# RyanXLi/OneshotDet

Measured on AMD Instinct MI355X. Metric: images/sec/GPU fwd+bwd, 800x1024 target + 127x127 query, bs=8; 1->8 GPU scaling, higher is better.
Workload: dtype bf16; 1 GPU; BASELINE.json configs[2]: bs=8/GPU, 800x1024 target + 127x127 query, bf16 MFMA convs, forward (two R-50-FPN backbones, query pooling, correlation, FCOS head, training proposals) + FCOS loss + backward (stem/layer1 frozen) + gradient all-reduce + SGD(momentum) + weight repack; global_batch=8, parallelism=dp1: one rank, no collective anywhere in the step, world_size=1

## Files before the change

include/oneshotdet_hip.h:

```cpp
#ifndef ONESHOTDET_HIP_H
#define ONESHOTDET_HIP_H

#include <stdint.h>

#ifdef __cplusplus
extern "C" {
#endif

#define OSD_F32 0
#define OSD_BF16 1

#define OSD_OK 0
#define OSD_ERR_INVALID_ARG (-1)
#define OSD_ERR_UNSUPPORTED (-2)
#define OSD_ERR_LAUNCH (-3)
#define OSD_ERR_WORKSPACE (-4)

#define OSD_ACT_NONE 0
#define OSD_ACT_RELU 1
#define OSD_ACT_EXP_SCALE 2

#define OSD_RES_NONE 0
#define OSD_RES_SAME 1
#define OSD_RES_UP2X 2
// ... 118 lines not shown
int osd_sigmoid_focal_bwd(const float* logits, const int32_t* targets, const float* d_losses, float* d_logits, int m,
                          int classes, float gamma, float alpha, void* stream);

int osd_pack_conv_weight_dgrad(const float* w, const float* scale, void* dst, int cout, int cin, int r, int s, int rows,
                               int cout_pad, int src_orsi, int dtype, void* stream);
int osd_conv2d_wgrad(const osd_conv_desc* d, const void* x, const void* dy, const float* scale, float* dw, float* db,
                     void* stream);
int osd_conv2d_wgrad_grouped(const osd_conv_desc* d, int n_seg, const void* const* xs, const void* const* dys,
                             const int32_t* ns, const int32_t* hs, const int32_t* ws, const float* scale, float* dw,
                             float* db, void* stream);
int osd_conv2d_wgrad_pred(const osd_conv_desc* d, int n_seg, const void* const* xs, const void* const* dys, const int32_t* ns,
                          const int32_t* hs, const int32_t* ws, float* dw, float* db, void* workspace, void* stream);
int64_t osd_conv2d_wgrad_pred_workspace_bytes(int n_seg, const int32_t* ns, const int32_t* hs, const int32_t* ws, int cin);
int osd_pred_dy_gather(const osd_conv_desc* d, int n_seg, const void* const* dys, const int32_t* ns, const int32_t* hs,
                       const int32_t* ws, void* g, void* stream);
int osd_pred_dgrad_pack(int dtype, const float* w, int cout, int cin, void* wd, void* stream);
int osd_conv2d_wgrad_pred_gathered(const osd_conv_desc* d, int n_seg, const void* const* xs, const void* g, const int32_t* ns,
                                   const int32_t* hs, const int32_t* ws, float* dw, float* db, void* workspace, void* stream);
int osd_conv2d_wgrad_batched(const osd_conv_desc* d, int n_seg, const void* const* xs, const void* const* dys,
                             const float* const* scales, float* const* dws, float* const* dbs, void* stream);
int osd_conv2d_wgrad_multi(const osd_conv_desc* d, int n_seg, const void* const* xs, const void* const* dys,
                           const int32_t* ns, const int32_t* hs, const int32_t* ws, const float* const* scales,
                           float* const* dws, float* const* dbs, void* stream);
int osd_conv2d_wgrad_mixed(int n_seg, const osd_conv_desc* descs, const void* const* xs, const void* const* dys,
                           const float* const* scales, float* const* dws, float* const* dbs, void* stream);
int osd_unpack_wgrad(const float* dw_packed, const float* scale, float* grad_oihw, int cout, int cin, int r, int s,
                     int accumulate, void* stream);
int osd_bias_grad(const void* dy, float* db, int m, int c, int stride, int dtype, void* stream);
int osd_conv2d_dgrad_naive(const osd_conv_desc* d, const void* dy, const void* w_fwd_packed, const void* mask,
                           const void* addend, void* dx, void* stream);
int osd_scatter2x(const void* src, const void* mask, const void* addend, void* dst, int n, int h, int w, int ho, int wo,
                  int c, int dtype, void* stream);
int osd_add_mask(const void* a, const void* b, const void* mask, void* out, int64_t numel, int dtype, void* stream);
int osd_upsample2x_bwd(const void* inner, const void* prev, void* top, int n, int h, int w, int c, int dtype, void* stream);
int osd_correlate_bwd_query(const void* g, const void* feat, float* dq, int n, int hw, int c, int dtype, void* stream);
int osd_correlate_bwd_query_levels(int n_levels, const void* const* gs, const void* const* feats, float* const* dqs,
                                   const int32_t* hws, int n, int c, int dtype, void* stream);
int osd_roialign_bwd(const float* gy, const float* rois, float* gx, int b, int h, int w, int c, int num_rois,
                     float spatial_scale, int ph, int pw, int sampling_ratio, void* stream);
int osd_shot_mean_bwd(const float* gy, float* gx, int b, int shots, int c, void* stream);
int osd_query_pool_levels_bwd(int n_levels, const float* const* dqs, const int32_t* hs, const int32_t* ws, const float* scales,
                              const float* rois, int batch, int shots, int c, int sampling_ratio, float* gx32, void* const* outs,
                              int dtype, void* stream);
int osd_query_avgpool_levels_bwd(int n_levels, const float* const* dqs, const int32_t* hs, const int32_t* ws, int batch,
                                 int shots, int c, void* const* outs, int dtype, void* stream);
int osd_cast_f32(const float* src, void* dst, int64_t numel, int dtype, void* stream);
int osd_grad_wire_cast(const void* src, void* dst, int64_t numel, int to_wire, void* stream);
int osd_sgd_momentum_multi(const void* table, const int32_t* block_entry, int n_blocks, float* params,
                           const float* grads, float* momentum_buf, float lr, float momentum, int first_step,
                           void* stream);
int osd_sgd_momentum_pack_multi(const void* table, const int32_t* block_entry, int n_blocks, float* params,
                                float* grads, float* momentum_buf, const float* scales, void* packed, int dtype,
                                float lr, float momentum, int first_step, int zero_grads, void* stream);
int osd_groupnorm_relu_fwd_levels(int n_levels, const void* const* xs, void* const* ys, const int32_t* hws,
                                  const float* gamma, const float* beta, float* ab, float* ws, int n, int c, int groups,
                                  float eps, int dtype, void* stream);
int osd_groupnorm_relu_fwd_levels_fused(int n_levels, const void* const* xs, void* const* ys, const int32_t* hws,
                                        const float* gamma, const float* beta, float* ab, float* ws, int n, int c, int groups,
                                        float eps, int dtype, uint32_t fused_mask, void* stream);
int64_t osd_groupnorm_onepass_workspace_bytes(int n_levels, const int32_t* hws, int n, int c, int groups, int backward);
int64_t osd_groupnorm_onepass_sync_bytes(int n_levels, int n);
int osd_groupnorm_relu_fwd_levels_onepass(int n_levels, const void* const* xs, void* const* ys, const int32_t* hws,
                                          const float* gamma, const float* beta, float* ab, float* ws, int32_t* sync, int n, int c,
                                          int groups, float eps, int dtype, void* stream);
int osd_groupnorm_relu_bwd_levels_onepass(int n_levels, const void* const* us, const void* const* dts, void* const* dus,
                                          const int32_t* hws, const float* ab, const float* gamma, const float* beta, float* ws,
                                          int32_t* sync, float* dgamma, float* dbeta, int n, int c, int groups, int dtype, void* stream);
int osd_groupnorm_onepass_selftest_timeout(int n_levels, const void* const* xs, void* const* ys, const int32_t* hws,
                                           const float* gamma, const float* beta, float* ab, float* ws, int32_t* sync, int n, int c,
                                           int groups, float eps, int dtype, int spin_limit, void* stream);
int osd_groupnorm_relu_bwd_levels(int n_levels, const void* const* us, const void* const* dts, void* const* dus,
                                  const int32_t* hws, const float* ab, const float* gamma, const float* beta, float* ws,
                                  float* dgamma, float* dbeta, int n, int c, int groups, int dtype, void* stream);
int osd_groupnorm_relu_bwd_levels_fused(int n_levels, const void* const* us, const void* const* dts, void* const* dus,
                                        const int32_t* hws, const float* ab, const float* gamma, const float* beta, float* ws,
                                        float* dgamma, float* dbeta, int n, int c, int groups, int dtype, uint32_t fused_mask,
                                        void* stream);
int osd_groupnorm_relu_bwd_levels_convbias(int n_levels, const void* const* us, const void* const* dts, void* const* dus,
                                           const int32_t* hws, const float* ab, const float* gamma, const float* beta, float* ws,
                                           float* dgamma, float* dbeta, float* conv_dbias, int n, int c, int groups, int dtype,
                                           void* stream);
int osd_fcos_loss_level(int phase, const void* cls_ctr, const void* reg, const float* gt_boxes, const int32_t* gt_count,
                        int max_gt, int n, int h, int w, int stride, float size_lo, float size_hi, float radius,
                        float gamma, float alpha, const float* scale_dev, float* sums, void* d_cls_ctr, void* d_reg,
                        int grad_stride, float* d_scale_raw, int dtype, void* stream);
int osd_fcos_loss_levels(int phase, int n_levels, const void* const* cls_ctrs, const void* const* regs,
                         const float* gt_boxes, const int32_t* gt_count, int max_gt, int n, const int32_t* hs,
                         const int32_t* ws, const int32_t* strides, const float* size_lo, const float* size_hi, float radius,
                         float gamma, float alpha, const float* const* scale_devs, float* sums, void* const* d_cls_ctrs,
                         void* const* d_regs, int grad_stride, float* const* d_scale_raws, int dtype, void* stream);
int osd_fcos_loss_finalize(const float* sums, float* losses, int n, void* stream);
int osd_fcos_loss_finalize_scales(const float* sums, float* losses, int n, const float* d_scale_raw, const float* scales,
                                  float* d_scales, int n_levels, void* stream);

#define OSD_MAX_ROI_LEVELS 8
int osd_roi_pool_levels(int n_levels, const void* const* xs, const int32_t* hs, const int32_t* ws, const float* scales,
                        const float* boxes, const int32_t* counts, void* y, int n, int c, int max_rois, int pool,
                        int sampling_ratio, int y_stride, int32_t* level_out, int dtype, void* stream);
int osd_groupnorm_act_rois(const void* x, const void* addend, const float* gamma, const float* beta, void* y,
                           int n_samples, int hw, int c, int groups, float eps, float slope, int rois_per_add,
                           int add_stride, int add_offset, int dtype, void* stream);
int osd_box_decode(const void* pred, const float* rois, const int32_t* counts, float* scores, float* boxes,
                   float* logits_out, float* reg_out, int n, int max_rois, int shots, int pred_stride,
                   const float* reg_weights, float img_h, float img_w, const float* img_hw, float score_thresh, int dtype,
                   void* stream);
int osd_append_gt_boxes(const float* boxes, const float* scores, const int32_t* counts, const float* gt_boxes,
// ... 50 lines not shown
```

oneshotdet_amd/_lib.py:

```python
import ctypes as C
import os

_HERE = os.path.dirname(os.path.abspath(__file__))
LIB_PATH = os.environ.get("OSD_LIB_PATH") or os.path.join(_HERE, "lib", "liboneshotdet_hip.so")

OSD_F32, OSD_BF16 = 0, 1
ABI_VERSION = 4
ACT_NONE, ACT_RELU, ACT_EXP_SCALE = 0, 1, 2
RES_NONE, RES_SAME, RES_UP2X, RES_DOWN2X = 0, 1, 2, 3
GN_SPLITS = 64


class ConvDesc(C.Structure):
    _fields_ = [(n, C.c_int32) for n in (
        "dtype", "n", "h", "w", "cin", "in_stride_n", "in_stride_h", "in_stride_w", "ho", "wo", "cout", "r", "s",
        "stride_h", "stride_w", "pad_h", "pad_w", "w_rows", "out_stride", "res_mode", "res_h", "res_w", "res_stride",
        "act")] + [("act_scale", C.c_float), ("relu_in", C.c_int32), ("algo", C.c_int32), ("reserved0", C.c_int32),
                   ("ordered_ws", C.c_void_p), ("ordered_ws_bytes", C.c_int64)]


_p, _i, _f, _i64 = C.c_void_p, C.c_int, C.c_float, C.c_int64

SIGNATURES = {
    "osd_last_error_string": (C.c_char_p, []),
    "osd_abi_version": (_i, []),
    "osd_conv_algo_count": (_i, []),
    "osd_conv2d_fwd": (_i, [C.POINTER(ConvDesc), _p, _p, _p, _p, _p, _p, _p, _p, _p]),
    "osd_conv2d_fwd_grouped": (_i, [C.POINTER(ConvDesc), _i, _p, _p, _p, _p, _p, _p, _p, _p, _p, _p, _p]),
    "osd_conv2d_fwd_multi": (_i, [C.POINTER(ConvDesc), _i, _p, _p, _p, _p, _p, _p, _p, _p, _p, _p, _p]),
    "osd_conv2d_fwd_multi_gn": (_i, [C.POINTER(ConvDesc), _i, _p, _p, _p, _p, _p, _p, _p, _p, _p, _p, _p, _p, _i, _i, _p]),
    "osd_pack_conv_weight": (_i, [_p, _p, _p, _i, _i, _i, _i, _i, _i, _i, _p]),
    "osd_pack_stem_weight": (_i, [_p, _p, _p, _i, _i, _i, _p]),
    "osd_pack_image": (_i, [_p, _p, _i, _i, _i, _i, _i, _i, _i, _i, _p]),
    "osd_nhwc_to_nchw_f32": (_i, [_p, _p, _i, _i, _i, _i, _i, _i, _i, _p]),
    "osd_nchw_f32_to_nhwc": (_i, [_p, _p, _i, _i, _i, _i, _i, _p]),
    "osd_maxpool3x3s2_fwd": (_i, [_p, _p, _i, _i, _i, _i, _i, _i, _i, _p]),
    "osd_groupnorm_stats": (_i, [_p, _p, _i, _i, _i, _i, _i, _p]),
    "osd_groupnorm_finalize": (_i, [_p, _p, _p, _p, _p, _i, _i, _i, _i, _f, _p]),
    "osd_groupnorm_relu_apply": (_i, [_p, _p, _p, _p, _i, _i, _i, _i, _p]),
    "osd_roialign_fwd": (_i, [_p, _p, _p, _i, _i, _i, _i, _i, _f, _i, _i, _i, _i, _p]),
    "osd_shot_mean": (_i, [_p, _p, _i, _i, _i, _p]),
    "osd_query_pool_levels": (_i, [_i, _p, _p, _p, _p, _p, _i, _i, _i, _i, _p, _i, _p]),
    "osd_query_pool_levels_bwd": (_i, [_i, _p, _p, _p, _p, _p, _i, _i, _i, _i, _p, _p, _i, _p]),
    "osd_query_avgpool_workspace_bytes": (_i64, [_i, _p, _p, _i, _i]),
    "osd_query_avgpool_levels": (_i, [_i, _p, _p, _p, _i, _i, _i, _p, _p, _i64, _i, _p]),
    "osd_query_avgpool_levels_bwd": (_i, [_i, _p, _p, _p, _i, _i, _i, _p, _i, _p]),
    "osd_correlate_fwd": (_i, [_p, _p, _p, _i, _i, _i, _i, _p]),
    "osd_correlate_levels": (_i, [_i, _p, _p, _p, _p, _i, _i, _i, _p]),
    "osd_correlate_bwd_query_levels": (_i, [_i, _p, _p, _p, _p, _i, _i, _i, _p]),
    "osd_fcos_score_decode": (_i, [_p, _p, _p, _p, _i, _i, _i, _i, _i, _i, _i, _i, _f, _f, _i, _p]),
    "osd_fcos_score_decode_sizes": (_i, [_p, _p, _p, _p, _i, _i, _i, _i, _i, _i, _i, _i, _f, _f, _p, _i, _p]),
    "osd_level_topk": (_i, [_p, _p, _i, _i, _i, _i, _i, _p]),
    "osd_rank_sort_gather": (_i, [_p, _p, _i, _i, _i, _p, _p, _i, _i, _p, _p, _p, _p, _p]),
    "osd_nms_sorted": (_i, [_p, _p, _p, _i, _i, _f, _i, _i, _p, _p, _p, _p, _p, _p]),
    "osd_nms_workspace_bytes": (_i64, [_i, _i]),
    "osd_nms": (_i, [_p, _p, _i, _f, _i, _p, _p, _p, _p]),
    "osd_nms_single_workspace_bytes": (_i64, [_i]),
    "osd_sigmoid_focal_fwd": (_i, [_p, _p, _p, _i, _i, _f, _f, _p]),
    "osd_sigmoid_focal_bwd": (_i, [_p, _p, _p, _p, _i, _i, _f, _f, _p]),
    "osd_pack_conv_weight_dgrad": (_i, [_p, _p, _p, _i, _i, _i, _i, _i, _i, _i, _i, _p]),
    "osd_pack_conv_weight_ex": (_i, [_p, _p, _p, _i, _i, _i, _i, _i, _i, _i, _i, _p]),
    "osd_conv2d_wgrad": (_i, [C.POINTER(ConvDesc), _p, _p, _p, _p, _p, _p]),
    "osd_groupnorm_relu_fwd_levels": (_i, [_i, _p, _p, _p, _p, _p, _p, _p, _i, _i, _i, _f, _i, _p]),
    "osd_groupnorm_relu_fwd_levels_fused": (_i, [_i, _p, _p, _p, _p, _p, _p, _p, _i, _i, _i, _f, _i, C.c_uint32, _p]),
    "osd_groupnorm_relu_bwd_levels": (_i, [_i, _p, _p, _p, _p, _p, _p, _p, _p, _p, _p, _i, _i, _i, _i, _p]),
    "osd_groupnorm_relu_bwd_levels_fused": (_i, [_i, _p, _p, _p, _p, _p, _p, _p, _p, _p, _p, _i, _i, _i, _i, C.c_uint32, _p]),
    "osd_groupnorm_relu_bwd_levels_convbias": (_i, [_i, _p, _p, _p, _p, _p, _p, _p, _p, _p, _p, _p, _i, _i, _i, _i, _p]),
    "osd_groupnorm_onepass_workspace_bytes": (_i64, [_i, _p, _i, _i, _i, _i]),
    "osd_groupnorm_onepass_sync_bytes": (_i64, [_i, _i]),
    "osd_groupnorm_relu_fwd_levels_onepass": (_i, [_i, _p, _p, _p, _p, _p, _p, _p, _p, _i, _i, _i, _f, _i, _p]),
    "osd_groupnorm_relu_bwd_levels_onepass": (_i, [_i, _p, _p, _p, _p, _p, _p, _p, _p, _p, _p, _p, _i, _i, _i, _i, _p]),
    "osd_groupnorm_onepass_selftest_timeout": (_i, [_i, _p, _p, _p, _p, _p, _p, _p, _p, _i, _i, _i, _f, _i, _i, _p]),
    "osd_sgd_momentum_multi": (_i, [_p, _p, _i, _p, _p, _p, _f, _f, _i, _p]),
    "osd_sgd_momentum_pack_multi": (_i, [_p, _p, _i, _p, _p, _p, _p, _p, _i, _f, _f, _i, _i, _p]),
    "osd_pack_multi": (_i, [_p, _p, _i, _p, _p, _p, _i, _i, _p]),
    "osd_conv2d_wgrad_grouped": (_i, [C.POINTER(ConvDesc), _i, _p, _p, _p, _p, _p, _p, _p, _p, _p]),
    "osd_conv2d_wgrad_pred": (_i, [C.POINTER(ConvDesc), _i, _p, _p, _p, _p, _p, _p, _p, _p, _p]),
    "osd_conv2d_wgrad_pred_workspace_bytes": (_i64, [_i, _p, _p, _p, _i]),
    "osd_pred_dy_gather": (_i, [C.POINTER(ConvDesc), _i, _p, _p, _p, _p, _p, _p]),
    "osd_pred_dgrad_pack": (_i, [_i, _p, _i, _i, _p, _p]),
    "osd_conv2d_wgrad_pred_gathered": (_i, [C.POINTER(ConvDesc), _i, _p, _p, _p, _p, _p, _p, _p, _p, _p]),
    "osd_conv2d_wgrad_batched": (_i, [C.POINTER(ConvDesc), _i, _p, _p, _p, _p, _p, _p]),
    "osd_conv2d_wgrad_multi": (_i, [C.POINTER(ConvDesc), _i, _p, _p, _p, _p, _p, _p, _p, _p, _p]),
    "osd_conv2d_wgrad_mixed": (_i, [_i, C.POINTER(ConvDesc), _p, _p, _p, _p, _p, _p]),
    "osd_unpack_wgrad": (_i, [_p, _p, _p, _i, _i, _i, _i, _i, _p]),
    "osd_bias_grad": (_i, [_p, _p, _i, _i, _i, _i, _p]),
    "osd_conv2d_dgrad_naive": (_i, [C.POINTER(ConvDesc), _p, _p, _p, _p, _p, _p]),
    "osd_scatter2x": (_i, [_p, _p, _p, _p, _i, _i, _i, _i, _i, _i, _i, _p]),
    "osd_add_mask": (_i, [_p, _p, _p, _p, _i64, _i, _p]),
    "osd_upsample2x_bwd": (_i, [_p, _p, _p, _i, _i, _i, _i, _i, _p]),
    "osd_correlate_bwd_query": (_i, [_p, _p, _p, _i, _i, _i, _i, _p]),
    "osd_roialign_bwd": (_i, [_p, _p, _p, _i, _i, _i, _i, _i, _f, _i, _i, _i, _p]),
    "osd_shot_mean_bwd": (_i, [_p, _p, _i, _i, _i, _p]),
    "osd_cast_f32": (_i, [_p, _p, _i64, _i, _p]),
    "osd_grad_wire_cast": (_i, [_p, _p, _i64, _i, _p]),
    "osd_fcos_loss_level": (_i, [_i, _p, _p, _p, _p, _i, _i, _i, _i, _i, _f, _f, _f, _f, _f, _p, _p, _p, _p, _i, _p, _i, _p]),
    "osd_fcos_loss_levels": (_i, [_i, _i, _p, _p, _p, _p, _i, _i, _p, _p, _p, _p, _p, _f, _f, _f, _p, _p, _p, _p, _i, _p, _i, _p]),
    "osd_fcos_loss_finalize": (_i, [_p, _p, _i, _p]),
    "osd_fcos_loss_finalize_scales": (_i, [_p, _p, _i, _p, _p, _p, _i, _p]),
    "osd_roi_pool_levels": (_i, [_i, _p, _p, _p, _p, _p, _p, _p, _i, _i, _i, _i, _i, _i, _p, _i, _p]),
    "osd_groupnorm_act_rois": (_i, [_p, _p, _p, _p, _p, _i, _i, _i, _i, _f, _f, _i, _i, _i, _i, _p]),
    "osd_box_decode": (_i, [_p, _p, _p, _p, _p, _p, _p, _i, _i, _i, _i, _p, _f, _f, _p, _f, _i, _p]),
    "osd_append_gt_boxes": (_i, [_p, _p, _p, _p, _p, _p, _p, _p, _i, _i, _i, _p]),
    "osd_proposals_sort_nms": (_i, [_p, _p, _i, _i, _i, _p, _p, _i, _i, _f, _i, _i, _p, _p, _p, _p, _p]),
    "osd_proposals_sort_nms_hint": (_i, [_p, _p, _i, _i, _i, _p, _p, _i, _i, _f, _i, _i, _i, _p, _p, _p, _p, _p, _p]),
    "osd_proposals_workspace_bytes": (_i64, [_i, _i, _i, _i]),
    "osd_box_match_sample": (_i, [_p, _p, _p, _p, _p, _p, _i, _i, _i, _i, _f, _f, _p, _p, _p, _p, _p, _p, _p, _p, _p]),
    "osd_box_loss": (_i, [_p, _p, _p, _p, _i, _i, _i, _f, _f, _p, _p, _i, _i, _p]),
    "osd_voc_match": (_i, [_p, _p, _p, _p, _p, _p, _p, _p, _i, _i, _i, _f, _p, _p, _p]),
    "osd_voc_curves": (_i, [_p, _p, _p, _i, _p, _p, _p]),
    "osd_voc_ap": (_i, [_p, _p, _p, _p, _p, _i, _i, _p, _p]),
    "osd_coco_match": (_i, [_p, _p, _p, _p, _p, _p, _i, _i, _i, _p, _i, _p, _i, _p, _p, _p, _p]),
    "osd_groupnorm_act_rois_bwd": (_i, [_p, _p, _p, _p, _p, _p, _p, _p, _p, _i, _i, _i, _i, _f, _f, _i, _i, _i, _i, _p]),
    "osd_rois_sum": (_i, [_p, _p, _i, _i, _i64, _i, _p]),
    "osd_roi_pool_levels_bwd": (_i, [_i, _p, _p, _p, _p, _p, _p, _p, _i, _i, _i, _i, _i, _i, _i, _p]),
    "osd_image_transform": (_i, [_p, _i, _i, _i, _i, _i, _i, _p, _p, _p, _i, _i, _i, _i, _i, _i, _i, _p, _p]),
    "osd_image_transform_workspace_bytes": (_i64, [_i, _i, _i, _i]),
    "osd_image_transform_batch": (_i, [_i, _p, _p, _p, _p, _p, _p, _i, _p, _p, _p, _i, _i, _i, _i, _i, _i, _i, _p, _p]),
}

_lib = None


class OsdError(RuntimeError):
    pass


# ... 32 lines not shown
```

oneshotdet_amd/csrc/backward.hip:

```cpp
#include "osd_common.h"
#include "conv_params.h"

namespace {

constexpr int kMaxBlocks = 2048;
inline int grid_for(long long work, int threads) {
  long long b = (work + threads - 1) / threads;
  if (b < 1) b = 1;
  return (int)(b > kMaxBlocks ? kMaxBlocks : b);
}

template <typename T> struct Chunk;
template <> struct Chunk<float> {
  static constexpr int N = 4;
  float v[4];
  __device__ __forceinline__ void load(const float* p) {
    const float4 t = *reinterpret_cast<const float4*>(p);
    v[0] = t.x; v[1] = t.y; v[2] = t.z; v[3] = t.w;
  }
  __device__ __forceinline__ void store(float* p) const { *reinterpret_cast<float4*>(p) = make_float4(v[0], v[1], v[2], v[3]); }
};
template <> struct Chunk<__bf16> {
  static constexpr int N = 8;
  float v[8];
// ... 171 lines not shown
  long long off, numel;
  float lr_mult, wd;
  int first_block, n_blocks;
};

__global__ void __launch_bounds__(256) sgd_multi_kernel(const SgdEntry* __restrict__ table, const int* __restrict__ block_entry,
                                                        float* __restrict__ p, const float* __restrict__ g,
                                                        float* __restrict__ buf, float lr, float momentum, int first) {
  const SgdEntry e = table[block_entry[blockIdx.x]];
  const float step = lr * e.lr_mult;
  const long long stride = (long long)e.n_blocks * blockDim.x;
  const long long tid = (long long)(blockIdx.x - e.first_block) * blockDim.x + threadIdx.x;
  const long long n4 = (e.off & 3) == 0 ? (e.numel >> 2) : 0;
  f32x4* p4 = reinterpret_cast<f32x4*>(p + e.off);
  const f32x4* g4 = reinterpret_cast<const f32x4*>(g + e.off);
  f32x4* b4 = reinterpret_cast<f32x4*>(buf + e.off);
  for (long long i = tid; i < n4; i += stride) {
    const f32x4 w = p4[i], gr = g4[i];
    f32x4 m;
    if (first) {
#pragma unroll
      for (int k = 0; k < 4; ++k) m[k] = gr[k] + e.wd * w[k];
    } else {
      const f32x4 bb = b4[i];
#pragma unroll
      for (int k = 0; k < 4; ++k) m[k] = momentum * bb[k] + (gr[k] + e.wd * w[k]);
    }
    f32x4 o;
#pragma unroll
    for (int k = 0; k < 4; ++k) o[k] = w[k] - step * m[k];
    b4[i] = m;
    p4[i] = o;
  }
  for (long long i = n4 * 4 + tid; i < e.numel; i += stride) {
    const long long k = e.off + i;
    const float w = p[k];
    const float d = g[k] + e.wd * w;
    const float m = first ? d : momentum * buf[k] + d;
    buf[k] = m;
    p[k] = w - step * m;
  }
}

struct SgdPackEntry {
  long long off, numel;
  float lr_mult, wd;
  int first_block, n_blocks;
  long long dst_off;
  long long scale_off;
  int cin, rs, kpad, pad_;
};

template <typename T>
__global__ void __launch_bounds__(256) sgd_pack_multi_kernel(const SgdPackEntry* __restrict__ table, const int* __restrict__ block_entry,
                                                             float* __restrict__ p, float* __restrict__ g, float* __restrict__ buf,
                                                             const float* __restrict__ scales, T* __restrict__ packed, float lr,
                                                             float momentum, int first, int zero_grads) {
  const SgdPackEntry e = table[block_entry[blockIdx.x]];
  const float step = lr * e.lr_mult;
  const long long stride = (long long)e.n_blocks * blockDim.x;
  const long long tid = (long long)(blockIdx.x - e.first_block) * blockDim.x + threadIdx.x;
  const bool pack = e.dst_off >= 0;
  const long long n4 = ((e.off & 3) == 0 && (!pack || (e.cin & 3) == 0)) ? (e.numel >> 2) : 0;
  f32x4* p4 = reinterpret_cast<f32x4*>(p + e.off);
  f32x4* g4 = reinterpret_cast<f32x4*>(g + e.off);
  f32x4* b4 = reinterpret_cast<f32x4*>(buf + e.off);
  const float* sc = e.scale_off >= 0 ? scales + e.scale_off : nullptr;
  const int cin4 = e.cin >> 2;
  const long long row4 = (long long)e.rs * cin4;
  for (long long i = tid; i < n4; i += stride) {
    const f32x4 w = p4[i], gr = g4[i];
    f32x4 m;
    if (first) {
#pragma unroll
      for (int k = 0; k < 4; ++k) m[k] = gr[k] + e.wd * w[k];
    } else {
      const f32x4 bb = b4[i];
#pragma unroll
      for (int k = 0; k < 4; ++k) m[k] = momentum * bb[k] + (gr[k] + e.wd * w[k]);
    }
    f32x4 o;
#pragma unroll
    for (int k = 0; k < 4; ++k) o[k] = w[k] - step * m[k];
    b4[i] = m;
    p4[i] = o;
    if (zero_grads) g4[i] = f32x4{0.f, 0.f, 0.f, 0.f};
    if (pack) {
      const long long co = i / row4;
      const long long rem = i - co * row4;
      const int tap = (int)(rem / cin4), ci = ((int)(rem - (long long)tap * cin4)) << 2;
      const float f = sc ? sc[co] : 1.f;
      T* d = packed + e.dst_off + ((size_t)co * e.rs + tap) * e.kpad + ci;
      if constexpr (sizeof(T) == 2) {
        bf16x4 q;
#pragma unroll
        for (int k = 0; k < 4; ++k) q[k] = (__bf16)(o[k] * f);
        *reinterpret_cast<bf16x4*>(d) = q;
      } else {
        *reinterpret_cast<f32x4*>(d) = f32x4{o[0] * f, o[1] * f, o[2] * f, o[3] * f};
      }
    }
  }
  const long long row1 = (long long)e.rs * e.cin;
  for (long long i = n4 * 4 + tid; i < e.numel; i += stride) {
    const long long k = e.off + i;
    const float w = p[k];
    const float d = g[k] + e.wd * w;
    const float m = first ? d : momentum * buf[k] + d;
    const float o = w - step * m;
    buf[k] = m;
    p[k] = o;
    if (zero_grads) g[k] = 0.f;
    if (pack) {
      const long long co = i / row1;
      const long long rem = i - co * row1;
      const int tap = (int)(rem / e.cin), ci = (int)(rem - (long long)tap * e.cin);
      packed[e.dst_off + ((size_t)co * e.rs + tap) * e.kpad + ci] = from_f32<T>(o * (sc ? sc[co] : 1.f));
    }
  }
}

__global__ void unpack_wgrad_kernel(const float* __restrict__ dwp, const float* __restrict__ scale, float* __restrict__ g,
                                    int cout, int cin, int R, int S, int accumulate) {
  const long long total = (long long)cout * cin * R * S;
  for (long long i = blockIdx.x * (long long)blockDim.x + threadIdx.x; i < total; i += (long long)gridDim.x * blockDim.x) {
    const int s = (int)(i % S);
    long long t = i / S;
    const int r = (int)(t % R); t /= R;
    const int ci = (int)(t % cin);
    const int co = (int)(t / cin);
    float v = dwp[(((size_t)co * R + r) * S + s) * cin + ci];
    if (scale) v *= scale[co];
    g[i] = accumulate ? g[i] + v : v;
  }
}

template <typename T>
__global__ void scatter2x_kernel(const T* __restrict__ src, const T* __restrict__ mask, const T* __restrict__ addend,
                                 T* __restrict__ dst, int n, int h, int w, int ho, int wo, int c) {
  constexpr int E = Chunk<T>::N;
  const int cch = c / E;
  const long long total = (long long)n * h * w * cch;
  for (long long i = blockIdx.x * (long long)blockDim.x + threadIdx.x; i < total; i += (long long)gridDim.x * blockDim.x) {
    const int cc = (int)(i % cch);
    long long t = i / cch;
    const int x = (int)(t % w); t /= w;
    const int y = (int)(t % h);
    const int b = (int)(t / h);
    Chunk<T> v;
#pragma unroll
    for (int e = 0; e < E; ++e) v.v[e] = 0.f;
    if (!(x & 1) && !(y & 1) && (y >> 1) < ho && (x >> 1) < wo)
      v.load(src + (((size_t)b * ho + (y >> 1)) * wo + (x >> 1)) * c + cc * E);
    if (addend) {
      Chunk<T> a;
      a.load(addend + i * E);
#pragma unroll
      for (int e = 0; e < E; ++e) v.v[e] += a.v[e];
    }
    if (mask) {
      Chunk<T> m;
      m.load(mask + i * E);
#pragma unroll
      for (int e = 0; e < E; ++e) v.v[e] = m.v[e] > 0.f ? v.v[e] : 0.f;
    }
    v.store(dst + i * E);
  }
}

template <typename T>
__global__ void add_mask_kernel(const T* __restrict__ a, const T* __restrict__ b, const T* __restrict__ mask, T* __restrict__ out,
                                long long chunks) {
// ... 241 lines not shown
}

#define OSD_STREAM(s) reinterpret_cast<hipStream_t>(s)
#define OSD_DISPATCH_DTYPE(dtype, CALL_F32, CALL_BF16)                            \
  do {                                                                           \
    if ((dtype) == OSD_F32) { CALL_F32; }                                        \
    else if ((dtype) == OSD_BF16) { CALL_BF16; }                                 \
    else return osd_fail(OSD_ERR_INVALID_ARG, "bad dtype %d", (int)(dtype));     \
  } while (0)

extern "C" int osd_pack_conv_weight_dgrad(const float* w, const float* scale, void* dst, int cout, int cin, int r, int s,
                                          int rows, int cout_pad, int src_orsi, int dtype, void* stream) {
  if (!w || !dst || rows < cin || cout_pad < cout) return osd_fail(OSD_ERR_INVALID_ARG, "pack_dgrad: bad args");
  const int g = grid_for((long long)rows * r * s * cout_pad, 256);
  OSD_DISPATCH_DTYPE(dtype,
      hipLaunchKernelGGL(pack_dgrad_weight_kernel<float>, dim3(g), dim3(256), 0, OSD_STREAM(stream), w, scale, (float*)dst, cout, cin, r, s, rows, cout_pad, src_orsi),
      hipLaunchKernelGGL(pack_dgrad_weight_kernel<__bf16>, dim3(g), dim3(256), 0, OSD_STREAM(stream), w, scale, (__bf16*)dst, cout, cin, r, s, rows, cout_pad, src_orsi));
  return osd_check_launch("pack_dgrad_weight");
}

extern "C" int osd_pack_multi(const void* table, const int32_t* block_entry, int n_blocks, const float* src,
                              const float* scales, void* dst, int dgrad, int dtype, void* stream) {
  if (!table || !block_entry || !src || !dst) return osd_fail(OSD_ERR_INVALID_ARG, "pack_multi: null argument");
  if (n_blocks <= 0) return OSD_OK;
  OSD_DISPATCH_DTYPE(dtype,
      hipLaunchKernelGGL(pack_multi_kernel<float>, dim3(n_blocks), dim3(256), 0, OSD_STREAM(stream), (const PackEntry*)table, block_entry, src, scales, (float*)dst, dgrad),
      hipLaunchKernelGGL(pack_multi_kernel<__bf16>, dim3(n_blocks), dim3(256), 0, OSD_STREAM(stream), (const PackEntry*)table, block_entry, src, scales, (__bf16*)dst, dgrad));
  return osd_check_launch("pack_multi");
}

extern "C" int osd_sgd_momentum_multi(const void* table, const int32_t* block_entry, int n_blocks, float* params,
                                      const float* grads, float* momentum_buf, float lr, float momentum, int first_step,
                                      void* stream) {
  if (!table || !block_entry || !params || !grads || !momentum_buf) return osd_fail(OSD_ERR_INVALID_ARG, "sgd: null argument");
  if (n_blocks <= 0) return OSD_OK;
  hipLaunchKernelGGL(sgd_multi_kernel, dim3(n_blocks), dim3(256), 0, OSD_STREAM(stream), (const SgdEntry*)table, block_entry,
                     params, grads, momentum_buf, lr, momentum, first_step);
  return osd_check_launch("sgd_multi");
}

extern "C" int osd_sgd_momentum_pack_multi(const void* table, const int32_t* block_entry, int n_blocks, float* params,
                                           float* grads, float* momentum_buf, const float* scales, void* packed, int dtype,
                                           float lr, float momentum, int first_step, int zero_grads, void* stream) {
  if (!table || !block_entry || !params || !grads || !momentum_buf || !packed) return osd_fail(OSD_ERR_INVALID_ARG, "sgd_pack: null argument");
  if (n_blocks <= 0) return OSD_OK;
  OSD_DISPATCH_DTYPE(dtype,
      hipLaunchKernelGGL(sgd_pack_multi_kernel<float>, dim3(n_blocks), dim3(256), 0, OSD_STREAM(stream), (const SgdPackEntry*)table, block_entry,
                         params, grads, momentum_buf, scales, (float*)packed, lr, momentum, first_step, zero_grads),
      hipLaunchKernelGGL(sgd_pack_multi_kernel<__bf16>, dim3(n_blocks), dim3(256), 0, OSD_STREAM(stream), (const SgdPackEntry*)table, block_entry,
                         params, grads, momentum_buf, scales, (__bf16*)packed, lr, momentum, first_step, zero_grads));
  return osd_check_launch("sgd_pack_multi");
}

extern "C" int osd_unpack_wgrad(const float* dw_packed, const float* scale, float* grad_oihw, int cout, int cin, int r, int s,
                                int accumulate, void* stream) {
  if (!dw_packed || !grad_oihw) return osd_fail(OSD_ERR_INVALID_ARG, "unpack_wgrad: null argument");
  hipLaunchKernelGGL(unpack_wgrad_kernel, dim3(grid_for((long long)cout * cin * r * s, 256)), dim3(256), 0, OSD_STREAM(stream),
                     dw_packed, scale, grad_oihw, cout, cin, r, s, accumulate);
  return osd_check_launch("unpack_wgrad");
}

extern "C" int osd_scatter2x(const void* src, const void* mask, const void* addend, void* dst, int n, int h, int w, int ho,
                             int wo, int c, int dtype, void* stream) {
  const int e = dtype == OSD_BF16 ? 8 : 4;
  if (!src || !dst || c % e) return osd_fail(OSD_ERR_INVALID_ARG, "scatter2x: bad args");
  const int g = grid_for((long long)n * h * w * (c / e), 256);
  OSD_DISPATCH_DTYPE(dtype,
      hipLaunchKernelGGL(scatter2x_kernel<float>, dim3(g), dim3(256), 0, OSD_STREAM(stream), (const float*)src, (const float*)mask, (const float*)addend, (float*)dst, n, h, w, ho, wo, c),
      hipLaunchKernelGGL(scatter2x_kernel<__bf16>, dim3(g), dim3(256), 0, OSD_STREAM(stream), (const __bf16*)src, (const __bf16*)mask, (const __bf16*)addend, (__bf16*)dst, n, h, w, ho, wo, c));
  return osd_check_launch("scatter2x");
}

extern "C" int osd_add_mask(const void* a, const void* b, const void* mask, void* out, int64_t numel, int dtype, void* stream) {
  const int e = dtype == OSD_BF16 ? 8 : 4;
  if (!a || !out || numel % e) return osd_fail(OSD_ERR_INVALID_ARG, "add_mask: bad args");
  if (numel == 0) return OSD_OK;
  const int g = grid_for(numel / e, 256);
  OSD_DISPATCH_DTYPE(dtype,
      hipLaunchKernelGGL(add_mask_kernel<float>, dim3(g), dim3(256), 0, OSD_STREAM(stream), (const float*)a, (const float*)b, (const float*)mask, (float*)out, (long long)(numel / e)),
      hipLaunchKernelGGL(add_mask_kernel<__bf16>, dim3(g), dim3(256), 0, OSD_STREAM(stream), (const __bf16*)a, (const __bf16*)b, (const __bf16*)mask, (__bf16*)out, (long long)(numel / e)));
  return osd_check_launch("add_mask");
}

extern "C" int osd_upsample2x_bwd(const void* inner, const void* prev, void* top, int n, int h, int w, int c, int dtype,
                                  void* stream) {
  const int e = dtype == OSD_BF16 ? 8 : 4;
  if (!inner || !top || c % e) return osd_fail(OSD_ERR_INVALID_ARG, "upsample2x_bwd: bad args");
  const int g = grid_for((long long)n * h * w * (c / e), 256);
  OSD_DISPATCH_DTYPE(dtype,
      hipLaunchKernelGGL(upsample2x_bwd_kernel<float>, dim3(g), dim3(256), 0, OSD_STREAM(stream), (const float*)inner, (const float*)prev, (float*)top, n, h, w, c),
      hipLaunchKernelGGL(upsample2x_bwd_kernel<__bf16>, dim3(g), dim3(256), 0, OSD_STREAM(stream), (const __bf16*)inner, (const __bf16*)prev, (__bf16*)top, n, h, w, c));
  return osd_check_launch("upsample2x_bwd");
}

extern "C" int osd_correlate_bwd_query(const void* g, const void* feat, float* dq, int n, int hw, int c, int dtype, void* stream) {
  const int e = dtype == OSD_BF16 ? 8 : 4;
  if (!g || !feat || !dq || c % e || 256 % (c / e)) return osd_fail(OSD_ERR_INVALID_ARG, "correlate_bwd_query: bad args");
  hipError_t er = hipMemsetAsync(dq, 0, sizeof(float) * (size_t)n * c, OSD_STREAM(stream));
  if (er != hipSuccess) return osd_fail(OSD_ERR_LAUNCH, "correlate_bwd_query: memset failed");
  if (n == 0 || hw == 0) return OSD_OK;
  int slabs = (hw + 63) / 64;
  if (slabs > 512) slabs = 512;
  dim3 grid(slabs, n);
  OSD_DISPATCH_DTYPE(dtype,
      hipLaunchKernelGGL(correlate_bwd_q_kernel<float>, grid, dim3(256), 0, OSD_STREAM(stream), (const float*)g, (const float*)feat, dq, hw, c),
      hipLaunchKernelGGL(correlate_bwd_q_kernel<__bf16>, grid, dim3(256), 0, OSD_STREAM(stream), (const __bf16*)g, (const __bf16*)feat, dq, hw, c));
// ... 654 lines not shown
```

oneshotdet_amd/trace.py:

```python
from .tuner import _TUNING

TRACE = None


def rec(kind, **kw):
    if TRACE is not None and not _TUNING[0]:
        TRACE.append((kind, kw))
```

oneshotdet_amd/train_update.py:

```python
import os

import torch

from . import streams

from . import ops
from .ops import PackedConv


class Update(object):
    def _build_pack_tables(self):
        import numpy as np
        mult = 64 if self.dtype == torch.bfloat16 else 16
        tr = [c for c in self.convs.values() if c.trainable]
        scale_off, scales = {}, []
        off = 0
        for c in tr:
            if c.bn_scale is not None:
                scale_off[c.name] = off
                scales.append(c.bn_scale)
                off += c.cout
        self._flat_scale = torch.cat(scales) if scales else torch.zeros(1, device=self.device)
        base = self.flat_w.data_ptr()
        self._pack = {}
        for form in (0, 1):
            entries, dst_off = [], 0
            for c in tr:
                if form == 0:
                    rows, kpad = ops._round_up(c.cout, 16), ops._round_up(c.cin, mult)
                else:
                    rows, kpad = ops._round_up(c.cin, 16), ops._round_up(c.cout, mult)
                numel = rows * c.r * c.s * kpad
                nb = max(1, min(64, (numel + 256 * 16 - 1) // (256 * 16)))
                entries.append(dict(c=c, src=(c.w.data_ptr() - base) // 4, dst=dst_off, scale=scale_off.get(c.name, -1), rows=rows,
                                    kpad=kpad, nb=nb, numel=numel))
                dst_off += (numel + 63) // 64 * 64
            flat = torch.zeros(dst_off, device=self.device, dtype=self.dtype)
            tables = {}
            for bucket in self.exchange.ranges:
                sub = [e for e in entries if self._bucket_of(e["c"].w) == bucket]
                if not sub:
                    continue
                tab = np.zeros((len(sub), 7), dtype=np.int64)
                blocks = []
                for i, e in enumerate(sub):
                    c = e["c"]
                    tab[i, 0:3] = (e["src"], e["dst"], e["scale"])
                    tab[i, 3:7] = np.frombuffer(np.array([c.cout, c.cin, c.r, c.s, e["rows"], e["kpad"], len(blocks), e["nb"]],
                                                         dtype=np.int32).tobytes(), dtype=np.int64)
                    blocks += [i] * e["nb"]
                tables[bucket] = dict(table=torch.from_numpy(tab).to(self.device),
                                      blocks=torch.tensor(blocks, dtype=torch.int32, device=self.device), n=len(blocks))
            self._pack[form] = dict(flat=flat, tables=tables)
            if form == 0:
                self._pack_fwd_entry = {id(e["c"]): e for e in entries}
            for e in entries:
                c = e["c"]
                view = flat[e["dst"]:e["dst"] + e["numel"]].view(e["rows"], c.r, c.s, e["kpad"])
                if form == 0:
                    cout_store = ops._round_up(c.cout, 4)
                    if c.has_bias and c.cout % 16 == 0:
                        bias = c.b
                    else:
                        bias = torch.zeros(ops._round_up(cout_store, 16), device=self.device, dtype=torch.float32)
                        if c.bn_shift is not None:
                            bias[:c.cout] = c.bn_shift
                    c.pc = PackedConv(view, bias, c.cout, cout_store, e["rows"], e["kpad"], c.r, c.s, cin_real=c.cin)
                else:
                    zb = torch.zeros(ops._round_up(c.cin, 16), device=self.device, dtype=torch.float32)
                    c.pd = PackedConv(view, zb, c.cin, c.cin, e["rows"], e["kpad"], c.r, c.s, cin_real=c.cout)
        self._padded_bias = {}
        for c in tr:
            if c.has_bias and c.cout % 16 != 0:
                self._padded_bias.setdefault(self._bucket_of(c.w), []).append(c)

    def repack(self, buckets=None, forms=(0, 1)):
        for c in self.convs.values():
            if not c.trainable and c.pc is None:
                c.pc = ops.pack_conv(self._frozen_sd[c.name + ".weight"], bn=None if c.bn_scale is None else tuple(
                    self._frozen_sd[c.name.replace("conv", "bn").replace("downsample.0", "downsample.1") + k]
                    for k in (".weight", ".bias", ".running_mean", ".running_var")), dtype=self.dtype,
                    stem=c.name.endswith("stem.conv1"))
        if not hasattr(self, "_pack"):
            self._build_pack_tables()
        for bucket in (self.exchange.ranges if buckets is None else buckets):
            for form in forms:
                pk = self._pack[form]
                tb = pk["tables"].get(bucket)
                if tb is not None:
                    ops._lib.call("osd_pack_multi", ops._ptr(tb["table"]), ops._ptr(tb["blocks"]), tb["n"], ops._ptr(self.flat_w),
                                  ops._ptr(self._flat_scale), ops._ptr(pk["flat"]), form, ops._dt(pk["flat"]), ops._stream())
            for c in self._padded_bias.get(bucket, ()):
                c.pc.bias[:c.cout] = c.b

    def _build_sgd_table(self, weights, biases):
        import numpy as np
        base = self.flat_w.data_ptr()
        conv_of = {c.w.data_ptr(): c for c in self.convs.values() if c.trainable}
        rows = {name: [] for name in self.exchange.ranges}
        for group, lr_mult, wd in ((weights, 1.0, self.weight_decay), (biases, 2.0, 0.0)):
            for t in group:
                rows[self._bucket_of(t)].append(((t.data_ptr() - base) // 4, t.numel(), lr_mult, wd, conv_of.get(t.data_ptr())))
        fuse = os.environ.get("OSD_NO_FUSED_REPACK", "0") == "0"
        tables = {}
        for name, rs in rows.items():
            if not rs:
                continue
            fused = fuse
            tab = np.zeros((len(rs), 8 if fused else 4), dtype=np.int64)
            blocks = []
            for i, (off, n, lm, wd, c) in enumerate(rs):
                nb = max(1, min(64, (n + 256 * 16 - 1) // (256 * 16)))
                tab[i, 0], tab[i, 1] = off, n
                tab[i, 2] = np.frombuffer(np.array([lm, wd], dtype=np.float32).tobytes(), dtype=np.int64)[0]
                tab[i, 3] = np.frombuffer(np.array([len(blocks), nb], dtype=np.int32).tobytes(), dtype=np.int64)[0]
                if fused:
                    tab[i, 4] = tab[i, 5] = -1
                    if c is not None:
                        e = self._pack_fwd_entry[id(c)]
                        cout = n // (c.cin * c.r * c.s)
                        assert e["kpad"] >= c.cin and cout * c.cin * c.r * c.s == n, (name, i, e["kpad"], c.cin, n)
                        assert 0 <= e["dst"] and e["dst"] + cout * c.r * c.s * e["kpad"] <= self._pack[0]["flat"].numel(), (name, i)
                        tab[i, 4], tab[i, 5] = e["dst"], e["scale"]
                        tab[i, 6:8] = np.frombuffer(np.array([c.cin, c.r * c.s, e["kpad"], 0], dtype=np.int32).tobytes(), dtype=np.int64)
                blocks += [i] * nb
            tables[name] = dict(table=torch.from_numpy(tab).to(self.device), fused=fused,
                                blocks=torch.tensor(blocks, dtype=torch.int32, device=self.device), n=len(blocks))
        self._sgd = dict(tables=tables, buf=torch.zeros_like(self.flat_w), steps=0)

    def _update_bucket(self, name):
        sg = self._sgd
        tb = sg["tables"].get(name)
        fused = tb is not None and tb["fused"]
        if fused:
            pk = self._pack[0]["flat"]
            ops._lib.call("osd_sgd_momentum_pack_multi", ops._ptr(tb["table"]), ops._ptr(tb["blocks"]), tb["n"],
                          ops._ptr(self.flat_w), ops._ptr(self.flat_g), ops._ptr(sg["buf"]), ops._ptr(self._flat_scale), ops._ptr(pk),
                          ops._dt(pk), float(self.lr), float(self.momentum), int(sg["steps"] == 0), int(self.consume_grads), ops._stream())
            if self.consume_grads:
                self._zeroed.add(name)
        elif tb is not None:
            ops._lib.call("osd_sgd_momentum_multi", ops._ptr(tb["table"]), ops._ptr(tb["blocks"]), tb["n"],
                          ops._ptr(self.flat_w), ops._ptr(self.flat_g), ops._ptr(sg["buf"]), float(self.lr),
                          float(self.momentum), int(sg["steps"] == 0), ops._stream())
        self.repack([name], forms=(1,) if fused else (0, 1))
        self._updated.add(name)

    def optimizer_step(self):
        if self.opt is not None:
            self.opt.step()
            self.repack()
            return
        if self._overlap:
            main = streams.current()
            main.wait_stream(self.ustream)
            if self.exchange.comm is not None:
                main.wait_stream(self.exchange.comm)
        for name in self.exchange.ranges:
            if name not in self._updated:
                self._update_bucket(name)
        self._end_of_update()
        self._sgd["steps"] += 1

    def _end_of_update(self):
        self._updated = set()
        self._grads_clean = bool(self.consume_grads and self._zeroed >= set(self._sgd["tables"]))
        self._zeroed = set()
```

Baseline: 782.2 images/sec.

## Fuse dgrad weight repack into SGD momentum update kernel via LDS transpose

Adds a pack2 SGD kernel that applies the momentum update and writes both the forward-packed and the dgrad-packed (flipped, transposed) bf16 weights in one pass. A 64x65 shared-memory tile handles the transpose, so the separate dgrad pack_multi launch per bucket is no longer needed and fp32 weights are not re-read. Conv entries get tile-based block counts, and non-conv entries fall back to the flat path. This adds shared-memory traffic and syncthreads, and block counts may no longer match entry size for small convs.

```diff
diff --git a/include/oneshotdet_hip.h b/include/oneshotdet_hip.h
--- a/include/oneshotdet_hip.h
+++ b/include/oneshotdet_hip.h
@@ -194,6 +194,10 @@
 int osd_sgd_momentum_pack_multi(const void* table, const int32_t* block_entry, int n_blocks, float* params,
                                 float* grads, float* momentum_buf, const float* scales, void* packed, int dtype,
                                 float lr, float momentum, int first_step, int zero_grads, void* stream);
+int osd_sgd_momentum_pack2_multi(const void* table, const int32_t* block_entry, int n_blocks, float* params,
+                                 float* grads, float* momentum_buf, const float* scales, void* packed,
+                                 void* packed_dgrad, int dtype, float lr, float momentum, int first_step, int zero_grads,
+                                 void* stream);
 int osd_groupnorm_relu_fwd_levels(int n_levels, const void* const* xs, void* const* ys, const int32_t* hws,
                                   const float* gamma, const float* beta, float* ab, float* ws, int n, int c, int groups,
                                   float eps, int dtype, void* stream);
diff --git a/oneshotdet_amd/_lib.py b/oneshotdet_amd/_lib.py
--- a/oneshotdet_amd/_lib.py
+++ b/oneshotdet_amd/_lib.py
@@ -73,6 +73,7 @@
     "osd_groupnorm_onepass_selftest_timeout": (_i, [_i, _p, _p, _p, _p, _p, _p, _p, _p, _i, _i, _i, _f, _i, _i, _p]),
     "osd_sgd_momentum_multi": (_i, [_p, _p, _i, _p, _p, _p, _f, _f, _i, _p]),
     "osd_sgd_momentum_pack_multi": (_i, [_p, _p, _i, _p, _p, _p, _p, _p, _i, _f, _f, _i, _i, _p]),
+    "osd_sgd_momentum_pack2_multi": (_i, [_p, _p, _i, _p, _p, _p, _p, _p, _p, _i, _f, _f, _i, _i, _p]),
     "osd_pack_multi": (_i, [_p, _p, _i, _p, _p, _p, _i, _i, _p]),
     "osd_conv2d_wgrad_grouped": (_i, [C.POINTER(ConvDesc), _i, _p, _p, _p, _p, _p, _p, _p, _p, _p]),
     "osd_conv2d_wgrad_pred": (_i, [C.POINTER(ConvDesc), _i, _p, _p, _p, _p, _p, _p, _p, _p, _p]),
diff --git a/oneshotdet_amd/csrc/backward.hip b/oneshotdet_amd/csrc/backward.hip
--- a/oneshotdet_amd/csrc/backward.hip
+++ b/oneshotdet_amd/csrc/backward.hip
@@ -247,11 +247,9 @@
 };
 
 template <typename T>
-__global__ void __launch_bounds__(256) sgd_pack_multi_kernel(const SgdPackEntry* __restrict__ table, const int* __restrict__ block_entry,
-                                                             float* __restrict__ p, float* __restrict__ g, float* __restrict__ buf,
-                                                             const float* __restrict__ scales, T* __restrict__ packed, float lr,
-                                                             float momentum, int first, int zero_grads) {
-  const SgdPackEntry e = table[block_entry[blockIdx.x]];
+__device__ __forceinline__ void sgd_pack_flat(const SgdPackEntry& e, float* __restrict__ p, float* __restrict__ g,
+                                              float* __restrict__ buf, const float* __restrict__ scales, T* __restrict__ packed,
+                                              float lr, float momentum, int first, int zero_grads) {
   const float step = lr * e.lr_mult;
   const long long stride = (long long)e.n_blocks * blockDim.x;
   const long long tid = (long long)(blockIdx.x - e.first_block) * blockDim.x + threadIdx.x;
@@ -313,6 +311,156 @@
       packed[e.dst_off + ((size_t)co * e.rs + tap) * e.kpad + ci] = from_f32<T>(o * (sc ? sc[co] : 1.f));
     }
   }
+}
+
+template <typename T>
+__global__ void __launch_bounds__(256) sgd_pack_multi_kernel(const SgdPackEntry* __restrict__ table, const int* __restrict__ block_entry,
+                                                             float* __restrict__ p, float* __restrict__ g, float* __restrict__ buf,
+                                                             const float* __restrict__ scales, T* __restrict__ packed, float lr,
+                                                             float momentum, int first, int zero_grads) {
+  const SgdPackEntry e = table[block_entry[blockIdx.x]];
+  sgd_pack_flat<T>(e, p, g, buf, scales, packed, lr, momentum, first, zero_grads);
+}
+
+struct SgdPack2Entry {
+  SgdPackEntry f;
+  long long ddst_off;
+  int cout, R, S;
+  int drows, dkpad;
+  int pad_;
+};
+static_assert(sizeof(SgdPackEntry) == 64 && sizeof(SgdPack2Entry) == 96, "table entries are laid out by the host");
+
+template <typename T, bool VEC>
+__device__ __forceinline__ void sgd_pack2_tiles(const SgdPack2Entry& e2, float (*big)[65], float* __restrict__ p, float* __restrict__ g,
+                                                float* __restrict__ buf, const float* __restrict__ scales, T* __restrict__ packed,
+                                                T* __restrict__ packed_d, float lr, float momentum, int first, int zero_grads) {
+  const SgdPackEntry& e = e2.f;
+  constexpr int EP = 16 / (int)sizeof(T);
+  const float step = lr * e.lr_mult;
+  const float* sc = e.scale_off >= 0 ? scales + e.scale_off : nullptr;
+  float* w = p + e.off;
+  float* gw = g + e.off;
+  float* bw = buf + e.off;
+  T* fwd = packed + e.dst_off;
+  T* out = packed_d + e2.ddst_off;
+  const int R = e2.R, S = e2.S;
+  const int tci = (e2.drows + 63) / 64, tco = (e2.dkpad + 63) / 64;
+  const int ntiles = R * S * tci * tco;
+  for (int t = blockIdx.x - e.first_block; t < ntiles; t += e.n_blocks) {
+    const int cit = t % tci;
+    int u = t / tci;
+    const int ss = u % S; u /= S;
+    const int rr = u % R;
+    const int cot = u / R;
+    const int co0 = cot * 64, ci0 = cit * 64;
+    const int tap = (R - 1 - rr) * S + (S - 1 - ss);
+    const int ci = ci0 + (threadIdx.x & 15) * 4;
+    const int nv = e.cin - ci;
+    f32x4 x[4], gr[4], bb[4];
+    size_t at[4];
+    bool in[4];
+#pragma unroll
+    for (int j = 0; j < 4; ++j) {
+      const int co = co0 + (threadIdx.x >> 4) + 16 * j;
+      in[j] = co < e2.cout && nv > 0;
+      at[j] = (((size_t)co * R + (R - 1 - rr)) * S + (S - 1 - ss)) * e.cin + ci;
+      if constexpr (VEC) {
+        if (in[j]) {
+          x[j] = *reinterpret_cast<const f32x4*>(w + at[j]);
+          gr[j] = *reinterpret_cast<const f32x4*>(gw + at[j]);
+          if (!first) bb[j] = *reinterpret_cast<const f32x4*>(bw + at[j]);
+        }
+      }
+    }
+    __syncthreads();
+#pragma unroll
+    for (int j = 0; j < 4; ++j) {
+      f32x4 v = f32x4{0.f, 0.f, 0.f, 0.f};
+      if (in[j]) {
+        const int co = co0 + (threadIdx.x >> 4) + 16 * j;
+        const float f = sc ? sc[co] : 1.f;
+        T* d = fwd + ((size_t)co * e.rs + tap) * e.kpad + ci;
+        if constexpr (VEC) {
+          const f32x4 wv = x[j];
+          f32x4 m;
+          if (first) {
+#pragma unroll
+            for (int k = 0; k < 4; ++k) m[k] = gr[j][k] + e.wd * wv[k];
+          } else {
+#pragma unroll
+            for (int k = 0; k < 4; ++k) m[k] = momentum * bb[j][k] + (gr[j][k] + e.wd * wv[k]);
+          }
+          f32x4 o;
+#pragma unroll
+          for (int k = 0; k < 4; ++k) o[k] = wv[k] - step * m[k];
+          *reinterpret_cast<f32x4*>(bw + at[j]) = m;
+          *reinterpret_cast<f32x4*>(w + at[j]) = o;
+          if (zero_grads) *reinterpret_cast<f32x4*>(gw + at[j]) = f32x4{0.f, 0.f, 0.f, 0.f};
+          v = f32x4{o[0] * f, o[1] * f, o[2] * f, o[3] * f};
+          if constexpr (sizeof(T) == 2) {
+            bf16x4 q;
+#pragma unroll
+            for (int k = 0; k < 4; ++k) q[k] = (__bf16)v[k];
+            *reinterpret_cast<bf16x4*>(d) = q;
+          } else {
+            *reinterpret_cast<f32x4*>(d) = v;
+          }
+        } else {
+#pragma unroll
+          for (int k = 0; k < 4; ++k) {
+            if (k < nv) {
+              const size_t i = at[j] + k;
+              const float wv = w[i];
+              const float dd = gw[i] + e.wd * wv;
+              const float m = first ? dd : momentum * bw[i] + dd;
+              const float o = wv - step * m;
+              bw[i] = m;
+              w[i] = o;
+              if (zero_grads) gw[i] = 0.f;
+              v[k] = o * f;
+              d[k] = from_f32<T>(v[k]);
+            }
+          }
+        }
+      }
+      float* trow = &big[(threadIdx.x >> 4) + 16 * j][(threadIdx.x & 15) * 4];
+      trow[0] = v[0]; trow[1] = v[1]; trow[2] = v[2]; trow[3] = v[3];
+    }
+    __syncthreads();
+    constexpr int CPW = 64 / EP;
+#pragma unroll
+    for (int j = 0; j < (64 * CPW) / 256; ++j) {
+      const int idx = threadIdx.x + 256 * j;
+      const int cr = ci0 + idx / CPW, cc = (idx % CPW) * EP;
+      if (cr >= e2.drows || co0 + cc >= e2.dkpad) continue;
+      T* o = out + (((size_t)cr * R + rr) * S + ss) * e2.dkpad + co0 + cc;
+      if constexpr (sizeof(T) == 2) {
+        bf16x8 v;
+#pragma unroll
+        for (int q = 0; q < 8; ++q) v[q] = (__bf16)big[cc + q][idx / CPW];
+        *reinterpret_cast<bf16x8*>(o) = v;
+      } else {
+        *reinterpret_cast<f32x4*>(o) = f32x4{big[cc][idx / CPW], big[cc + 1][idx / CPW], big[cc + 2][idx / CPW], big[cc + 3][idx / CPW]};
+      }
+    }
+  }
+}
+
+template <typename T>
+__global__ void __launch_bounds__(256) sgd_pack2_multi_kernel(const SgdPack2Entry* __restrict__ table, const int* __restrict__ block_entry,
+                                                              float* __restrict__ p, float* __restrict__ g, float* __restrict__ buf,
+                                                              const float* __restrict__ scales, T* __restrict__ packed,
+                                                              T* __restrict__ packed_d, float lr, float momentum, int first,
+                                                              int zero_grads) {
+  __shared__ float big[64][65];
+  const SgdPack2Entry e2 = table[block_entry[blockIdx.x]];
+  if (e2.ddst_off < 0 || e2.f.dst_off < 0)
+    sgd_pack_flat<T>(e2.f, p, g, buf, scales, packed, lr, momentum, first, zero_grads);
+  else if ((e2.f.cin & 3) == 0 && (e2.f.off & 3) == 0)
+    sgd_pack2_tiles<T, true>(e2, big, p, g, buf, scales, packed, packed_d, lr, momentum, first, zero_grads);
+  else
+    sgd_pack2_tiles<T, false>(e2, big, p, g, buf, scales, packed, packed_d, lr, momentum, first, zero_grads);
 }
 
 __global__ void unpack_wgrad_kernel(const float* __restrict__ dwp, const float* __restrict__ scale, float* __restrict__ g,
@@ -660,6 +808,21 @@
   return osd_check_launch("sgd_pack_multi");
 }
 
+extern "C" int osd_sgd_momentum_pack2_multi(const void* table, const int32_t* block_entry, int n_blocks, float* params,
+                                            float* grads, float* momentum_buf, const float* scales, void* packed,
+                                            void* packed_dgrad, int dtype, float lr, float momentum, int first_step,
+                                            int zero_grads, void* stream) {
+  if (!table || !block_entry || !params || !grads || !momentum_buf || !packed || !packed_dgrad)
+    return osd_fail(OSD_ERR_INVALID_ARG, "sgd_pack2: null argument");
+  if (n_blocks <= 0) return OSD_OK;
+  OSD_DISPATCH_DTYPE(dtype,
+      hipLaunchKernelGGL(sgd_pack2_multi_kernel<float>, dim3(n_blocks), dim3(256), 0, OSD_STREAM(stream), (const SgdPack2Entry*)table, block_entry,
+                         params, grads, momentum_buf, scales, (float*)packed, (float*)packed_dgrad, lr, momentum, first_step, zero_grads),
+      hipLaunchKernelGGL(sgd_pack2_multi_kernel<__bf16>, dim3(n_blocks), dim3(256), 0, OSD_STREAM(stream), (const SgdPack2Entry*)table, block_entry,
+                         params, grads, momentum_buf, scales, (__bf16*)packed, (__bf16*)packed_dgrad, lr, momentum, first_step, zero_grads));
+  return osd_check_launch("sgd_pack2_multi");
+}
+
 extern "C" int osd_unpack_wgrad(const float* dw_packed, const float* scale, float* grad_oihw, int cout, int cin, int r, int s,
                                 int accumulate, void* stream) {
   if (!dw_packed || !grad_oihw) return osd_fail(OSD_ERR_INVALID_ARG, "unpack_wgrad: null argument");
diff --git a/oneshotdet_amd/trace.py b/oneshotdet_amd/trace.py
--- a/oneshotdet_amd/trace.py
+++ b/oneshotdet_amd/trace.py
@@ -6,3 +6,11 @@
 def rec(kind, **kw):
     if TRACE is not None and not _TUNING[0]:
         TRACE.append((kind, kw))
+
+
+UPDATES = None
+
+
+def rec_update(kind, **kw):
+    if UPDATES is not None and not _TUNING[0]:
+        UPDATES.append((kind, kw))
diff --git a/oneshotdet_amd/train_update.py b/oneshotdet_amd/train_update.py
--- a/oneshotdet_amd/train_update.py
+++ b/oneshotdet_amd/train_update.py
@@ -5,12 +5,12 @@
 from . import streams
 
 from . import ops
+from . import trace
 from .ops import PackedConv
 
 
 class Update(object):
     def _build_pack_tables(self):
-        import numpy as np
         mult = 64 if self.dtype == torch.bfloat16 else 16
         tr = [c for c in self.convs.values() if c.trainable]
         scale_off, scales = {}, []
@@ -39,21 +39,13 @@
             tables = {}
             for bucket in self.exchange.ranges:
                 sub = [e for e in entries if self._bucket_of(e["c"].w) == bucket]
-                if not sub:
-                    continue
-                tab = np.zeros((len(sub), 7), dtype=np.int64)
-                blocks = []
-                for i, e in enumerate(sub):
-                    c = e["c"]
-                    tab[i, 0:3] = (e["src"], e["dst"], e["scale"])
-                    tab[i, 3:7] = np.frombuffer(np.array([c.cout, c.cin, c.r, c.s, e["rows"], e["kpad"], len(blocks), e["nb"]],
-                                                         dtype=np.int32).tobytes(), dtype=np.int64)
-                    blocks += [i] * e["nb"]
-                tables[bucket] = dict(table=torch.from_numpy(tab).to(self.device),
-                                      blocks=torch.tensor(blocks, dtype=torch.int32, device=self.device), n=len(blocks))
+                if sub:
+                    tables[bucket] = self._pack_table(sub)
             self._pack[form] = dict(flat=flat, tables=tables)
             if form == 0:
                 self._pack_fwd_entry = {id(e["c"]): e for e in entries}
+            else:
+                self._pack_dgrad_entry = {id(e["c"]): e for e in entries}
             for e in entries:
                 c = e["c"]
                 view = flat[e["dst"]:e["dst"] + e["numel"]].view(e["rows"], c.r, c.s, e["kpad"])
@@ -74,6 +66,19 @@
             if c.has_bias and c.cout % 16 != 0:
                 self._padded_bias.setdefault(self._bucket_of(c.w), []).append(c)
 
+    def _pack_table(self, sub):
+        import numpy as np
+        tab = np.zeros((len(sub), 7), dtype=np.int64)
+        blocks = []
+        for i, e in enumerate(sub):
+            c = e["c"]
+            tab[i, 0:3] = (e["src"], e["dst"], e["scale"])
+            tab[i, 3:7] = np.frombuffer(np.array([c.cout, c.cin, c.r, c.s, e["rows"], e["kpad"], len(blocks), e["nb"]],
+                                                 dtype=np.int32).tobytes(), dtype=np.int64)
+            blocks += [i] * e["nb"]
+        return dict(table=torch.from_numpy(tab).to(self.device),
+                    blocks=torch.tensor(blocks, dtype=torch.int32, device=self.device), n=len(blocks))
+
     def repack(self, buckets=None, forms=(0, 1)):
         for c in self.convs.values():
             if not c.trainable and c.pc is None:
@@ -88,6 +93,7 @@
                 pk = self._pack[form]
                 tb = pk["tables"].get(bucket)
                 if tb is not None:
+                    trace.rec_update("pack_multi_dgrad" if form else "pack_multi_fwd", bucket=bucket, n_blocks=tb["n"])
                     ops._lib.call("osd_pack_multi", ops._ptr(tb["table"]), ops._ptr(tb["blocks"]), tb["n"], ops._ptr(self.flat_w),
                                   ops._ptr(self._flat_scale), ops._ptr(pk["flat"]), form, ops._dt(pk["flat"]), ops._stream())
             for c in self._padded_bias.get(bucket, ()):
@@ -102,15 +108,27 @@
             for t in group:
                 rows[self._bucket_of(t)].append(((t.data_ptr() - base) // 4, t.numel(), lr_mult, wd, conv_of.get(t.data_ptr())))
         fuse = os.environ.get("OSD_NO_FUSED_REPACK", "0") == "0"
+        dpack = fuse and os.environ.get("OSD_NO_SGD_DPACK", "0") == "0"
         tables = {}
         for name, rs in rows.items():
             if not rs:
                 continue
             fused = fuse
-            tab = np.zeros((len(rs), 8 if fused else 4), dtype=np.int64)
+            tab = np.zeros((len(rs), 12 if dpack else 8 if fused else 4), dtype=np.int64)
             blocks = []
             for i, (off, n, lm, wd, c) in enumerate(rs):
                 nb = max(1, min(64, (n + 256 * 16 - 1) // (256 * 16)))
+                d = self._pack_dgrad_entry[id(c)] if dpack and c is not None else None
+                if d is not None:
+                    assert d["src"] == off and d["rows"] >= c.cin and d["kpad"] >= c.cout, (name, i)
+                    assert d["kpad"] % (16 // self._pack[1]["flat"].element_size()) == 0, (name, i, d["kpad"])
+                    assert 0 <= d["dst"] and d["dst"] + d["numel"] <= self._pack[1]["flat"].numel(), (name, i)
+                    nb = max(1, min(64, c.r * c.s * ((d["rows"] + 63) // 64) * ((d["kpad"] + 63) // 64)))
+                    tab[i, 8] = d["dst"]
+                    tab[i, 9:12] = np.frombuffer(np.array([c.cout, c.r, c.s, d["rows"], d["kpad"], 0], dtype=np.int32).tobytes(),
+                                                 dtype=np.int64)
+                elif dpack:
+                    tab[i, 8] = -1
                 tab[i, 0], tab[i, 1] = off, n
                 tab[i, 2] = np.frombuffer(np.array([lm, wd], dtype=np.float32).tobytes(), dtype=np.int64)[0]
                 tab[i, 3] = np.frombuffer(np.array([len(blocks), nb], dtype=np.int32).tobytes(), dtype=np.int64)[0]
@@ -124,7 +142,7 @@
                         tab[i, 4], tab[i, 5] = e["dst"], e["scale"]
                         tab[i, 6:8] = np.frombuffer(np.array([c.cin, c.r * c.s, e["kpad"], 0], dtype=np.int32).tobytes(), dtype=np.int64)
                 blocks += [i] * nb
-            tables[name] = dict(table=torch.from_numpy(tab).to(self.device), fused=fused,
+            tables[name] = dict(table=torch.from_numpy(tab).to(self.device), fused=fused, dpack=dpack,
                                 blocks=torch.tensor(blocks, dtype=torch.int32, device=self.device), n=len(blocks))
         self._sgd = dict(tables=tables, buf=torch.zeros_like(self.flat_w), steps=0)
 
@@ -134,16 +152,23 @@
         fused = tb is not None and tb["fused"]
         if fused:
             pk = self._pack[0]["flat"]
-            ops._lib.call("osd_sgd_momentum_pack_multi", ops._ptr(tb["table"]), ops._ptr(tb["blocks"]), tb["n"],
-                          ops._ptr(self.flat_w), ops._ptr(self.flat_g), ops._ptr(sg["buf"]), ops._ptr(self._flat_scale), ops._ptr(pk),
-                          ops._dt(pk), float(self.lr), float(self.momentum), int(sg["steps"] == 0), int(self.consume_grads), ops._stream())
+            tail = (float(self.lr), float(self.momentum), int(sg["steps"] == 0), int(self.consume_grads), ops._stream())
+            head = (ops._ptr(tb["table"]), ops._ptr(tb["blocks"]), tb["n"], ops._ptr(self.flat_w), ops._ptr(self.flat_g),
+                    ops._ptr(sg["buf"]), ops._ptr(self._flat_scale), ops._ptr(pk))
+            if tb["dpack"]:
+                trace.rec_update("sgd_pack2_multi", bucket=name, n_blocks=tb["n"])
+                ops._lib.call("osd_sgd_momentum_pack2_multi", *head, ops._ptr(self._pack[1]["flat"]), ops._dt(pk), *tail)
+            else:
+                trace.rec_update("sgd_pack_multi", bucket=name, n_blocks=tb["n"])
+                ops._lib.call("osd_sgd_momentum_pack_multi", *head, ops._dt(pk), *tail)
             if self.consume_grads:
                 self._zeroed.add(name)
         elif tb is not None:
+            trace.rec_update("sgd_multi", bucket=name, n_blocks=tb["n"])
             ops._lib.call("osd_sgd_momentum_multi", ops._ptr(tb["table"]), ops._ptr(tb["blocks"]), tb["n"],
                           ops._ptr(self.flat_w), ops._ptr(self.flat_g), ops._ptr(sg["buf"]), float(self.lr),
                           float(self.momentum), int(sg["steps"] == 0), ops._stream())
-        self.repack([name], forms=(1,) if fused else (0, 1))
+        self.repack([name], forms=() if fused and tb["dpack"] else (1,) if fused else (0, 1))
         self._updated.add(name)
 
     def optimizer_step(self):
```

Result: no change. 780.5 images/sec (median of 2 runs) (-0.2%).
